# pixray/pixray

Measured on AMD Instinct MI355X. Metric: optimisation iters/sec, VQGAN 256^2 + ViT-B/32 + 64 cutouts, higher is better.
Workload: dtype fp16

## Files before the change

### include/prx.h

```cpp
#ifndef PRX_H_
#define PRX_H_
#include <stddef.h>
#include <stdint.h>

#ifdef __cplusplus
extern "C" {
#endif

#define PRX_ABI_VERSION 3

typedef void* prx_stream_t;

const char* prx_last_error(void);
int prx_abi_version(void);
int prx_device_info(int* cu_count, char* arch_name, int arch_name_len);


#define PRX_ACT_NONE 0
#define PRX_ACT_QUICKGELU 1
#define PRX_ACT_MUL_DQUICKGELU 2
#define PRX_ACT_RELU 3
#define PRX_ACT_MUL_RELUMASK 4
#define PRX_ACT_RELUMASK_POST 5
#define PRX_ACT_GELU 6
// ... 14 lines not shown
    int a_is_f32, a_mode, lda;
    const void* B;
    int ldb;
    int M, N, K;
    int H, W, Cin, up;
    float alpha;
    const float* bias_n;
    const float* bias_m;
    const void* aux;
    int ldaux;
    const float* resid;
    int ldr;
    int act;
    float* out_f32; int ldc_f32;
    void* out_bf16; void* out_bf16_pre; int ldc_bf16;
    int f32;
    int row16;
    prx_gemm_ctx* ctx;
} prx_gemm_args;
int prx_k_gemm(const prx_gemm_args* g, void* ws, size_t ws_bytes, prx_stream_t stream);
int prx_k_gemm_gn(const prx_gemm_args* g, double* gn_stats, int gn_gs, const float* gnb_x, const double* gnb_fstats,
                  const float* gnb_gamma, const float* gnb_beta, int gnb_swish, float gnb_eps, void* ws, size_t ws_bytes,
                  prx_stream_t stream);
long long prx_gemm_fit_spec_launches(void);
long long prx_gemm_row_launches(void);

int prx_k_groupnorm_fwd(const float* x, const float* gamma, const float* beta, double* stats, void* out_bf16,
                        float* out_f32, int NB, int P, int C, int swish, float eps, prx_stream_t s);
int prx_k_groupnorm_bwd(const float* g, const float* x, const float* gamma, const float* beta, const double* fstats,
                        double* bstats, const float* add, float* dx, int NB, int P, int C, int swish, float eps,
                        prx_stream_t s);
int prx_k_layernorm_fwd(const float* x, long long ldx, const float* gamma, const float* beta, void* out_bf16,
                        float* out_f32, float* mean, float* rstd, int rows, int C, float eps, prx_stream_t s);
int prx_k_layernorm_bwd(const float* g, long long ldg, const float* x, long long ldx, const float* gamma,
                        const float* mean, const float* rstd, const float* add, long long ldadd, float* dx,
                        long long lddx, int rows, int C, prx_stream_t s);
int prx_k_transpose_bf16(const void* in, int ldin, void* out, int ldout, int R, int C, prx_stream_t s);
int prx_k_softmax_rows(const float* S, int lds_, float scale, void* P, int ldp, void* PT, int ldpt, int rows, int cols,
                       prx_stream_t s);
int prx_k_softmax_rows_bwd(const void* P, int ldp, const float* dP, int lddp, float scale, void* dS, int ldds,
                           void* dST, int lddst, int rows, int cols, prx_stream_t s);
int prx_k_upsample2x_bwd(const float* hi, float* low, int NB, int Hl, int Wl, int C, prx_stream_t s);
int prx_k_nchw_to_nhwc(const float* in, float* out_f32, void* out_bf16, int NB, int C, int HW, int Cpad,
                       prx_stream_t s);
int prx_k_nhwc_to_nchw(const float* in, int ldc, float* out, int NB, int C, int HW, prx_stream_t s);
int prx_k_image_head_fwd(const float* x, int ldc, float* img, int NB, int C, int HW, prx_stream_t s);
// ... 73 lines not shown
int prx_k_warp_a_bwd(const float* g, int Hs, int Ws, const double* desc, float* uv, float* gsrc_priv, float* gsrc, int n_cut, int Ha,
                     int Wa, int form, prx_stream_t s);
int prx_k_warp_b_fwd(const float* a, int Ha, int Wa, const double* desc, const float* noise, float* out, int n_cut, int S,
                     prx_stream_t s);
int prx_k_warp_b_bwd(const float* a, int Ha, int Wa, const double* desc, const float* g, float* grgb, float* uv, float* ga, int n_cut,
                     int S, float* maps_scratch, size_t maps_scratch_bytes, int form, prx_stream_t s);
int prx_k_vgg_pack(const float* w, void* Wf, void* Wd, int Cout, int Cin, int CiP, int prec, prx_stream_t s);
int prx_k_vgg_input(const float* x, void* out, int HW, int prec, prx_stream_t s);
int prx_k_vgg_input_grad(const float* d, float* gx, int HW, const float* unscale, prx_stream_t s);
int prx_k_vgg_maxpool(const void* x, void* out, void* arg, int H, int W, int C, int prec, prx_stream_t s);
int prx_k_vgg_combine(const float* above, const void* arg, const float* gcap, const void* act, void* gpre, int H, int W, int C,
                      const float* gscale, int prec, prx_stream_t s);
int prx_k_pack_transpose_op(const float* in, void* out, int R, int C, int prec, prx_stream_t s);
int prx_k_vit_add_cls_pos(float* x, const float* cls, const float* pos, int N, int T, int W, prx_stream_t s);
int prx_k_vit_embed_tokens(const float* x, const float* cls, const float* pos, void* out, int out16, int N, int T, int W,
                           prx_stream_t s);
int prx_k_vit_gelu_f32(const float* t, float* io, size_t n, int bwd, prx_stream_t s);
int prx_k_vit_scale_f32(float* x, size_t n, float scale, int blocks, prx_stream_t s);
int prx_k_text_embed(const int* tokens, const float* emb, const float* pos, float* x, int* eot, int n, int ctx, int W, int vocab,
                     prx_stream_t s);
int prx_k_gather_rows(const float* x, const int* eot, float* out, int n, int ctx, int W, prx_stream_t s);
int prx_k_l2norm_fwd(const float* e, float* out, int n, int D, prx_stream_t s);
int prx_k_l2norm_bwd(const float* e, const float* g, float* de, int n, int D, prx_stream_t s);
int prx_k_vqgan_pack_conv3x3(const float* w, void* Wf, void* Wd, int Cout, int Cin, int CoP, int prec, prx_stream_t s);
int prx_k_vqgan_enc_pack_conv3x3(const float* w, void* Wf, int Cout, int Cin, int CiP, prx_stream_t s);
int prx_k_colminmax(const float* w, float* mn, float* mx, int rows, int D, prx_stream_t s);


typedef struct prx_vqgan prx_vqgan;
typedef struct prx_vqgan_config {
    int ch;
    int ch_mult[8];
    int n_mult;
    int num_res_blocks;
    int attn_resolution;
    int resolution;
    int z_channels;
    int embed_dim;
    int n_embed;
    int out_ch;
    int latent_h, latent_w;
    int precision;
} prx_vqgan_config;
int prx_vqgan_create(prx_vqgan** out, const prx_vqgan_config* cfg, const float* const* weights, int n_weights,
                     prx_stream_t s);
void prx_vqgan_destroy(prx_vqgan* h);
// ... 277 lines not shown
```

### pixray_amd/csrc/api_core.hip

```cpp
#include "common.h"
#include "gemm.h"
#include "../../include/prx.h"
#include <stdarg.h>
#include <stdio.h>
#include <string.h>
#include <stdlib.h>

static thread_local char g_err[1024] = "";

void prx_set_error(const char* fmt, ...) {
    va_list ap;
    va_start(ap, fmt);
    vsnprintf(g_err, sizeof(g_err), fmt, ap);
    va_end(ap);
}

int prx_xcd_local() {
    static const int v = getenv("PRX_XCD_LOCAL") ? atoi(getenv("PRX_XCD_LOCAL")) : 1;
    return v;
}

int prx_grad_target_log2() {
    static const int v = [] {
        const char* e = getenv("PRX_GRAD_TARGET_LOG2");
// ... 38 lines not shown
    d.out_f32 = g->out_f32; d.ldc_f32 = g->ldc_f32;
    d.out_bf16 = g->out_bf16; d.out_bf16_pre = g->out_bf16_pre;
    d.ldc_bf16 = g->ldc_bf16;
    d.row16 = (short)(g->row16 & 3);
    return 0;
}
int prx_k_gemm(const prx_gemm_args* g, void* ws, size_t ws_bytes, prx_stream_t stream_) {
    GemmDesc d;
    int r = desc_of(g, d);
    if (r) return r;
    return prx_gemm_launch(d, (float*)ws, ws_bytes, (hipStream_t)stream_, (GemmCtx*)g->ctx);
}
int prx_k_gemm_gn(const prx_gemm_args* g, double* gn_stats, int gn_gs, const float* gnb_x, const double* gnb_fstats,
                  const float* gnb_gamma, const float* gnb_beta, int gnb_swish, float gnb_eps, void* ws, size_t ws_bytes,
                  prx_stream_t stream_) {
    GemmDesc d;
    int r = desc_of(g, d);
    if (r) return r;
    PRX_REQUIRE(gn_stats != nullptr, "prx_k_gemm_gn: null gn_stats");
    d.gn_stats = gn_stats; d.gn_gs = gn_gs;
    d.gnb_x = gnb_x; d.gnb_fstats = gnb_fstats; d.gnb_gamma = gnb_gamma; d.gnb_beta = gnb_beta; d.gnb_swish = gnb_swish; d.gnb_eps = gnb_eps;
    return prx_gemm_launch(d, (float*)ws, ws_bytes, (hipStream_t)stream_, (GemmCtx*)g->ctx);
}

prx_gemm_ctx* prx_gemm_ctx_create(void) { return (prx_gemm_ctx*)new GemmCtx(); }
void prx_gemm_ctx_destroy(prx_gemm_ctx* c) { delete (GemmCtx*)c; }
void prx_profile_gemm_enable(prx_gemm_ctx* c, int on) { prx_gemm_ctx_profile_enable((GemmCtx*)c, on); }
void prx_gemm_tile_override(prx_gemm_ctx* c, int bm, int bn, int splits) { prx_gemm_ctx_force_tile((GemmCtx*)c, bm, bn, splits); }
int prx_gemm_plan(prx_gemm_ctx* c, const prx_gemm_args* g, size_t ws_bytes, int n_cu, int* out) {
    GemmDesc d;
    int r = desc_of(g, d);
    if (r) return r;
    GemmPlan p;
    r = prx_gemm_plan_impl(d, (const GemmCtx*)c, n_cu, ws_bytes, true, &p);
    if (r) return r;
    const GemmLaunchPlan& l0 = p.launch[0], l1 = p.n_launch == 2 ? p.launch[1] : GemmLaunchPlan{};
    const int o[9] = {l0.family, l0.bm, l0.bn, l0.splits, p.rows_8p, p.n_launch == 2 ? (int)l1.family : -1, l1.bm, l1.bn, p.n_launch == 2 ? l1.splits : 0};
    memcpy(out, o, sizeof o);
    return 0;
}
int prx_gemm_plan_rows_8phase(prx_gemm_ctx* c, int M, int N, int K) {
    if (M <= 0 || N <= 0 || K <= 0) return 0;
    prx_gemm_args g = {};
    g.a_mode = PRX_A_ROWMAJOR; g.lda = g.ldb = K; g.M = M; g.N = N; g.K = K; g.alpha = 1.f;
    int out[9];
    return prx_gemm_plan(c, &g, 0, c ? ((GemmCtx*)c)->n_cu : 0, out) == 0 ? out[4] : 0;
// ... 10 lines not shown
```

### pixray_amd/csrc/api_kernels.hip

```cpp
#include "common.h"
#include "norms.h"
#include "elementwise.h"
#include "attention.h"
#include "resnet.h"
#include "cutouts.h"
#include "vgg.h"
#include "vit.h"
#include "clip_text.h"
#include "prompt_vq.h"
#include "vqgan.h"
#include "vqgan_enc.h"
#include "../../include/prx.h"

#define S_(x) ((hipStream_t)(x))
#define B_(x) ((bf16_t*)(x))
#define CB_(x) ((const bf16_t*)(x))

extern "C" {

int prx_k_groupnorm_fwd(const float* x, const float* gamma, const float* beta, double* stats, void* out_bf16,
                        float* out_f32, int NB, int P, int C, int swish, float eps, prx_stream_t s) {
    return prx_groupnorm_fwd(x, gamma, beta, stats, B_(out_bf16), out_f32, NB, P, C, swish, eps, S_(s));
}
int prx_k_groupnorm_bwd(const float* g, const float* x, const float* gamma, const float* beta, const double* fstats,
// ... 272 lines not shown
    return prx_vit_add_cls_pos(x, cls, pos, N, T, W, S_(s));
}
int prx_k_vit_embed_tokens(const float* x, const float* cls, const float* pos, void* out, int out16, int N, int T, int W, prx_stream_t s) {
    return prx_vit_embed_tokens(x, cls, pos, out, out16, N, T, W, S_(s));
}
int prx_k_vit_gelu_f32(const float* t, float* io, size_t n, int bwd, prx_stream_t s) {
    return prx_vit_gelu_f32(t, io, n, bwd, S_(s));
}
int prx_k_vit_scale_f32(float* x, size_t n, float scale, int blocks, prx_stream_t s) {
    return prx_vit_scale_f32(x, n, scale, blocks, S_(s));
}
int prx_k_text_embed(const int* tokens, const float* emb, const float* pos, float* x, int* eot, int n, int ctx, int W, int vocab, prx_stream_t s) {
    return prx_text_embed(tokens, emb, pos, x, eot, n, ctx, W, vocab, S_(s));
}
int prx_k_gather_rows(const float* x, const int* eot, float* out, int n, int ctx, int W, prx_stream_t s) {
    return prx_gather_rows(x, eot, out, n, ctx, W, S_(s));
}
int prx_k_l2norm_fwd(const float* e, float* out, int n, int D, prx_stream_t s) {
    return prx_l2norm_fwd(e, out, n, D, S_(s));
}
int prx_k_l2norm_bwd(const float* e, const float* g, float* de, int n, int D, prx_stream_t s) {
    return prx_l2norm_bwd(e, g, de, n, D, S_(s));
}
int prx_k_vqgan_pack_conv3x3(const float* w, void* Wf, void* Wd, int Cout, int Cin, int CoP, int prec, prx_stream_t s) {
    return prx_vqgan_pack_conv3x3(w, Wf, Wd, Cout, Cin, CoP, prec, S_(s));
}
int prx_k_vqgan_enc_pack_conv3x3(const float* w, void* Wf, int Cout, int Cin, int CiP, prx_stream_t s) {
    return prx_vqgan_enc_pack_conv3x3(w, Wf, Cout, Cin, CiP, S_(s));
}
int prx_k_colminmax(const float* w, float* mn, float* mx, int rows, int D, prx_stream_t s) {
    return prx_colminmax(w, mn, mx, rows, D, S_(s));
}

}
```

### pixray_amd/csrc/gemmfit.hip

```cpp
#include "gemmfit_kernel.h"
#include <atomic>

static std::atomic<long long> g_spec_launches{0};

namespace {
struct FitTile { int bm, bn, ks, tn; double eff; };
const FitTile kFitTiles[] = {
    {160, 256, 1, 64, 1.00}, {160, 192, 1, 48, 0.97}, {256, 128, 1, 64, 0.95}, {160, 128, 1, 32, 0.90}, {128, 128, 1, 32, 0.85},
    {80, 128, 2, 32, 0.85}, {128, 64, 2, 32, 0.75}, {64, 64, 2, 32, 0.60}, {32, 64, 4, 32, 0.45}, {16, 64, 4, 32, 0.35}, {16, 32, 8, 32, 0.25},
    {256, 16, 1, 16, 0.20},
};
const FitTile* fit_tile(int bm, int bn) {
    for (const FitTile& t : kFitTiles)
        if (t.bm == bm && t.bn == bn) return &t;
    return nullptr;
}
}

bool prx_gemmfit_tile(int bm, int bn, int* ks) {
    const FitTile* t = fit_tile(bm, bn);
    if (ks) *ks = t ? t->ks : 0;
    return t != nullptr;
}
bool prx_gemmfit_eligible(const GemmDesc& d, int bm, int bn) {
// ... 48 lines not shown
        if (!prx_gemmfit_eligible(d, tbm, tbn)) return;
        const int tm_ = ceil_div(d.M, tbm), tn_ = ceil_div(d.N, tbn);
        const int wgs = tm_ * tn_;
        if (wgs > 2 * n_cu) return;
        const double fill = (double)wgs / ((double)ceil_div(wgs, n_cu) * n_cu);
        const double waste = ((double)tm_ * tbm / d.M) * ((double)tn_ * tbn / d.N);
        const double score = fill * eff / waste;
        if (score > best && fill / waste >= 0.8) { best = score; *bm = tbm; *bn = tbn; }
    };
    if (d.a_mode == PRX_A_CONV3X3 && d.N <= 16 && d.M >= 4096 && prx_gemmfit_eligible(d, 256, 16)) { *bm = 256; *bn = 16; return; }
    if ((long long)d.M * d.N <= 256ll * 512 && d.K >= 512 && d.N >= 32) {
        if (prx_gemmfit_eligible(d, 16, 32)) { *bm = 16; *bn = 32; return; }
        if (d.N >= 64 && prx_gemmfit_eligible(d, 16, 64)) { *bm = 16; *bn = 64; return; }
    }
    for (const FitTile& t : kFitTiles)
        if (t.bn >= 32) consider(t.bm, t.bn, t.eff);
}
extern std::atomic<long long> g_prx_gemm8p_spec_launches;
extern "C" long long prx_gemm_fit_spec_launches(void) {
    return g_spec_launches.load(std::memory_order_relaxed) + g_prx_gemm8p_spec_launches.load(std::memory_order_relaxed);
}

int prx_gemmfit_epi_kind(const GemmDesc& d) {
    if (!d.h16 || d.f32 || d.a_is_f32 || d.out_f32 || !d.out_bf16 || d.bias_m) return FIT_EPI_GENERIC;
    const unsigned long long lim = 1ull << 31;
    if ((unsigned long long)d.M * d.ldc_bf16 >= lim || (d.resid && (unsigned long long)d.M * d.ldr >= lim) ||
        (d.aux && (unsigned long long)d.M * d.ldaux >= lim) || (unsigned long long)d.M * d.N >= lim) return FIT_EPI_GENERIC;
    const bool stats = d.gn_stats != nullptr, gnb = d.gnb_x != nullptr;
    if (gnb && !stats) return FIT_EPI_GENERIC;
    switch (d.act) {
    case PRX_ACT_NONE:
        if (d.aux) return FIT_EPI_GENERIC;
        if (gnb) return (!d.resid && (d.row16 & 2)) ? FIT_EPI_GNB : FIT_EPI_GENERIC;
        if (d.resid) return (d.row16 & 1) ? (stats ? FIT_EPI_RES16_GN : FIT_EPI_RES16) : FIT_EPI_GENERIC;
        return stats ? FIT_EPI_GN : FIT_EPI_OUT16;
    case PRX_ACT_QUICKGELU:
        return (d.out_bf16_pre && !d.resid && !stats) ? FIT_EPI_GELU : FIT_EPI_GENERIC;
    case PRX_ACT_MUL_DQUICKGELU:
        return (d.aux && !d.resid && !stats) ? FIT_EPI_DGELU : FIT_EPI_GENERIC;
    default:
        return FIT_EPI_GENERIC;
    }
}
#ifdef PRX_FIT_TRACE
namespace {
unsigned long long* g_trace_buf = nullptr;
size_t g_trace_cap = 0, g_trace_used = 0;
// ... 64 lines not shown
```

### pixray_amd/csrc/gemmfit_kernel.h

```cpp
#pragma once
#include "gemm_epi.h"
#include <type_traits>
#include <algorithm>
#include <stdlib.h>
#include <string>
#include <string.h>
#include <stdio.h>

const bf16_t* prx_gemm_zero_page();
int prx_gemmfit_epi_kind(const GemmDesc& d);
bool prx_gemmfit_launch_spec_tower(const prx_gemm_dev::GemmArgs& a, int bm, int bn, int epi, dim3 grid, hipStream_t s, const bf16_t* zp);
bool prx_gemmfit_launch_spec_dec_a(const prx_gemm_dev::GemmArgs& a, int bm, int bn, int epi, dim3 grid, hipStream_t s, const bf16_t* zp);
bool prx_gemmfit_launch_spec_dec_b(const prx_gemm_dev::GemmArgs& a, int bm, int bn, int epi, dim3 grid, hipStream_t s, const bf16_t* zp);
bool prx_gemmfit_launch_spec_dec_c(const prx_gemm_dev::GemmArgs& a, int bm, int bn, int epi, dim3 grid, hipStream_t s, const bf16_t* zp);
bool prx_gemmfit_launch_f32(const prx_gemm_dev::GemmArgs& a, int bm, int bn, dim3 grid, hipStream_t s, const bf16_t* zp);

namespace {
using namespace prx_gemm_dev;

constexpr int FIT_BK = 64;
constexpr int FIT_STAGES = 3;
typedef const __attribute__((address_space(1))) void* fit_gptr;
typedef __attribute__((address_space(3))) void* fit_lptr;

// ... 224 lines not shown
                    fit_gnb_accum(d, gc1, __builtin_bit_cast(float4, pf[ic][ps][1]), v1, gsb0, gsb1);
                } else if (do_stats) {
                    gsa0 += (v0.x + v0.y) + (v0.z + v0.w);
                    gsa1 += (v0.x * v0.x + v0.y * v0.y) + (v0.z * v0.z + v0.w * v0.w);
                    gsb0 += (v1.x + v1.y) + (v1.z + v1.w);
                    gsb1 += (v1.x * v1.x + v1.y * v1.y) + (v1.z * v1.z + v1.w * v1.w);
                }
            }
        }
    }
    FIT_TRACE(5);
    if (do_stats) fit_stats_tail<WGM, WGN, FN, KS>(d, fl + DUMP + 2 * NW * (16 * LDW), gsa0, gsa1, gsb0, gsb1, tn, kg, wm, wn, lane);
}

enum { FIT_EPI_GENERIC = 0,
       FIT_EPI_OUT16,
       FIT_EPI_RES16,
       FIT_EPI_GELU,
       FIT_EPI_DGELU,
       FIT_EPI_GN,
       FIT_EPI_RES16_GN,
       FIT_EPI_GNB,
       FIT_EPI_F32,
       FIT_EPI_COUNT };

__device__ __forceinline__ float fit_sigmoid(float x) { return __builtin_amdgcn_rcpf(1.f + __expf(-x)); }

template <int WGM, int WGN, int FM, int FN, int KS, int EPI>
__device__ __forceinline__ void fit_finish_spec(const GemmArgs& p, float* const fl, f32x4 (&acc)[FM][FN], int tm, int tn, int wave, int kg,
                                                int wt, int wm, int wn, int lane FIT_TRACE_ARG) {
    typedef __attribute__((ext_vector_type(8))) half_t h16x8;
    constexpr int NWT = WGM * WGN, NW = NWT * KS;
    constexpr int BM = 16 * FM * WGM, BN = 16 * FN * WGN, TN = 16 * FN;
    constexpr bool RESID = EPI == FIT_EPI_RES16 || EPI == FIT_EPI_RES16_GN;
    constexpr bool DGELU = EPI == FIT_EPI_DGELU, GELU = EPI == FIT_EPI_GELU, GNB = EPI == FIT_EPI_GNB;
    constexpr bool ROWOP = RESID || DGELU || GNB;
    constexpr bool STATS = EPI == FIT_EPI_GN || EPI == FIT_EPI_RES16_GN || GNB;
    static_assert(!STATS || BM % 80 != 0, "GroupNorm sums belong to the decoder's tiles");
    const GemmDesc& d = p.d;
    const int l15 = lane & 15, kq = lane >> 4;
    constexpr int DUMP = KS > 1 ? NW * FM * FN * 256 : 0;
    fit_ksum<WGM, WGN, FM, FN, KS>(fl, acc, kg, wt, lane);
    FIT_TRACE(4);

    constexpr int LDW = TN + 4, LPR = TN / 8, RPP = 64 / LPR, NPASS = (16 + RPP - 1) / RPP;
    constexpr int NOWN = (FM + KS - 1) / KS;
    constexpr int NBUF = NOWN > 1 ? 2 : 1, SLAB = 16 * LDW;
    float* const stage = fl + DUMP + wave * (2 * SLAB);
    const int rbase = tm * BM + wm * (16 * FM), cbase = tn * BN + wn * TN;
    const int lr0 = lane / LPR, lc = (lane - lr0 * LPR) * 8;
    const int col = cbase + lc;
    const bool col_ok = lane < RPP * LPR && col < d.N;
    const int colc = col_ok ? col : 0;
    const float alpha = d.alpha_dev ? d.alpha * *d.alpha_dev : d.alpha;
    float bias[8] = {0.f, 0.f, 0.f, 0.f, 0.f, 0.f, 0.f, 0.f};
    if (d.bias_n) {
        const float4 b0 = *reinterpret_cast<const float4*>(d.bias_n + colc), b1 = *reinterpret_cast<const float4*>(d.bias_n + colc + 4);
        bias[0] = b0.x; bias[1] = b0.y; bias[2] = b0.z; bias[3] = b0.w; bias[4] = b1.x; bias[5] = b1.y; bias[6] = b1.z; bias[7] = b1.w;
    }
    GnbConst gc0{}, gc1{};
    if constexpr (GNB) { gc0 = gnb_load(d, colc); gc1 = gnb_load(d, colc + 4); }
    const half_t* const rowp = RESID ? reinterpret_cast<const half_t*>(d.resid) : DGELU ? reinterpret_cast<const half_t*>(d.aux)
                                                                                      : reinterpret_cast<const half_t*>(d.gnb_x);
    const unsigned ldrow = RESID ? (unsigned)d.ldr : DGELU ? (unsigned)d.ldaux : (unsigned)d.N;
    half_t* const out = reinterpret_cast<half_t*>(d.out_bf16);
    half_t* const outp = reinterpret_cast<half_t*>(d.out_bf16_pre);
    const unsigned ldo = (unsigned)d.ldc_bf16;
    const int mlast = d.M - 1;

    uint4 pf[ROWOP ? FM : 1][NPASS];
    if constexpr (ROWOP) {
#pragma unroll
        for (int i = 0; i < FM; ++i) {
            if (KS > 1 && i % KS != kg) continue;
#pragma unroll
            for (int ps = 0; ps < NPASS; ++ps) {
                int lr = ps * RPP + lr0;
                lr = lr < 15 ? lr : 15;
                int row = rbase + i * 16 + lr;
                row = row < mlast ? row : mlast;
                pf[i][ps] = *reinterpret_cast<const uint4*>(rowp + ((unsigned)row * ldrow + (unsigned)colc));
            }
        }
    }

    float gsa0 = 0.f, gsa1 = 0.f, gsb0 = 0.f, gsb1 = 0.f;
    auto put = [&](int i, float* st) {
#pragma unroll
        for (int j = 0; j < FN; ++j)
#pragma unroll
// ... 20 lines not shown
                for (int e = 0; e < 8; ++e) x[e] = (float)rx[e];
            }
#pragma unroll
            for (int e = 0; e < 8; ++e) {
                v[e] *= alpha;
                v[e] += bias[e];
                if constexpr (DGELU) {
                    const float sg = fit_sigmoid(1.702f * x[e]);
                    v[e] *= sg * (1.f + 1.702f * x[e] * (1.f - sg));
                }
                if constexpr (RESID) v[e] += x[e];
            }
            const unsigned oo = (unsigned)row * ldo + (unsigned)col;
            if constexpr (GELU) {
                h16x8 q;
#pragma unroll
                for (int e = 0; e < 8; ++e) {
                    q[e] = f32_to_f16_sat(v[e]);
                    const float t = (float)q[e];
                    v[e] = t * fit_sigmoid(1.702f * t);
                }
                if (ok) *reinterpret_cast<h16x8*>(outp + oo) = q;
            }
            {
                h16x8 q;
#pragma unroll
                for (int e = 0; e < 8; ++e) q[e] = f32_to_f16_sat(v[e]);
                if (ok) *reinterpret_cast<h16x8*>(out + oo) = q;
            }
            if constexpr (GNB) {
                if (ok) {
                    fit_gnb_accum<true>(d, gc0, make_float4(x[0], x[1], x[2], x[3]), make_float4(v[0], v[1], v[2], v[3]), gsa0, gsa1);
                    fit_gnb_accum<true>(d, gc1, make_float4(x[4], x[5], x[6], x[7]), make_float4(v[4], v[5], v[6], v[7]), gsb0, gsb1);
                }
            } else if constexpr (STATS) {
                if (ok) {
                    gsa0 += (v[0] + v[1]) + (v[2] + v[3]);
                    gsa1 += (v[0] * v[0] + v[1] * v[1]) + (v[2] * v[2] + v[3] * v[3]);
                    gsb0 += (v[4] + v[5]) + (v[6] + v[7]);
                    gsb1 += (v[4] * v[4] + v[5] * v[5]) + (v[6] * v[6] + v[7] * v[7]);
                }
            }
        }
    }
    FIT_TRACE(5);
    if constexpr (STATS) fit_stats_tail<WGM, WGN, FN, KS>(d, fl + DUMP + 2 * NW * SLAB, gsa0, gsa1, gsb0, gsb1, tn, kg, wm, wn, lane);
}
// ... 424 lines not shown
```

### pixray_amd/csrc/gemmfit_spec_dec_c.hip

```cpp
#include "gemmfit_kernel.h"

#define DEC_TILE(...)                                                                     \
    switch (epi) {                                                                        \
        FIT_SPEC_CASE(FIT_EPI_OUT16, __VA_ARGS__, FIT_EPI_OUT16, true)                    \
        FIT_SPEC_CASE(FIT_EPI_RES16, __VA_ARGS__, FIT_EPI_RES16, true)                    \
        FIT_SPEC_CASE(FIT_EPI_GN, __VA_ARGS__, FIT_EPI_GN, true)                          \
        FIT_SPEC_CASE(FIT_EPI_RES16_GN, __VA_ARGS__, FIT_EPI_RES16_GN, true)              \
        FIT_SPEC_CASE(FIT_EPI_GNB, __VA_ARGS__, FIT_EPI_GNB, true)                        \
        default: return false;                                                            \
    }

bool prx_gemmfit_launch_spec_dec_c(const prx_gemm_dev::GemmArgs& a, int bm, int bn, int epi, dim3 grid, hipStream_t s, const bf16_t* zp) {
    if (bm == 32 && bn == 64) { DEC_TILE(1, 2, 2, 2, 4) }
    if (bm == 16 && bn == 64) { DEC_TILE(1, 2, 1, 2, 4) }
    if (bm == 16 && bn == 32) { DEC_TILE(1, 1, 1, 2, 8) }
    return false;
}
```

### pixray_amd/csrc/gemmfit_spec_tower.hip

```cpp
#include "gemmfit_kernel.h"

#define TOWER_TILE(...)                                                                   \
    switch (epi) {                                                                        \
        FIT_SPEC_CASE(FIT_EPI_OUT16, __VA_ARGS__, FIT_EPI_OUT16, false)                   \
        FIT_SPEC_CASE(FIT_EPI_RES16, __VA_ARGS__, FIT_EPI_RES16, false)                   \
        FIT_SPEC_CASE(FIT_EPI_GELU, __VA_ARGS__, FIT_EPI_GELU, false)                     \
        FIT_SPEC_CASE(FIT_EPI_DGELU, __VA_ARGS__, FIT_EPI_DGELU, false)                   \
        default: return false;                                                            \
    }

bool prx_gemmfit_launch_spec_tower(const prx_gemm_dev::GemmArgs& a, int bm, int bn, int epi, dim3 grid, hipStream_t s, const bf16_t* zp) {
    if (a.d.a_mode != PRX_A_ROWMAJOR) return false;
    if (bm == 160 && bn == 256) { TOWER_TILE(2, 4, 5, 4, 1) }
    if (bm == 160 && bn == 192) { TOWER_TILE(2, 4, 5, 3, 1) }
    if (bm == 160 && bn == 128) { TOWER_TILE(2, 4, 5, 2, 1) }
    if (bm == 80 && bn == 128) { TOWER_TILE(1, 4, 5, 2, 2) }
    return false;
}
```

### pixray_amd/csrc/prompt_vq.h

```cpp
#pragma once
#include "common.h"
int prx_prompt_loss(const float* x, const float* embed, int n, int m, int D, float weight, float stop, float denom,
                    float* rowloss, float* grad, float* loss, unsigned* ticket, hipStream_t s);
int prx_l2norm_fwd(const float* e, float* out, int n, int D, hipStream_t s);
int prx_l2norm_bwd(const float* e, const float* g, float* de, int n, int D, hipStream_t s);
int prx_sqnorm_rows(const float* w, float* out, int rows, int D, hipStream_t s);
int prx_vq_nearest(const float* z, long long tok_stride, long long ch_stride, const float* codebook, const float* cnorm,
                   int P, int NC, int D, float* pmin, int* pidx, int* idx_out, float* zq, hipStream_t s);
```

### pixray_amd/csrc/prompt_vq.hip

```cpp
#include "prompt_vq.h"
#include <algorithm>

namespace {

__device__ __forceinline__ float prompt_loss_row(const float* __restrict__ x, const float* __restrict__ embed, int i, int lane,
                                                int n, int m, int D, float weight, float stop, float denom,
                                                float* __restrict__ rowloss, float* __restrict__ grad) {
    constexpr int MAXE = 16;
    const int ne = D / 64;
    float xv[MAXE], gacc[MAXE];
    float ss = 0.f;
#pragma unroll
    for (int e = 0; e < MAXE; ++e) xv[e] = x[(size_t)i * D + (e < ne ? e : 0) * 64 + lane];
#pragma unroll
    for (int e = 0; e < MAXE; ++e)
        if (e < ne) { ss += xv[e] * xv[e]; gacc[e] = 0.f; }
    const float xnorm = fmaxf(sqrtf(wave_sum(ss)), 1e-12f);
    const float ixn = 1.f / xnorm;
    const float sgn = (weight > 0.f) ? 1.f : ((weight < 0.f) ? -1.f : 0.f);
    float loss = 0.f;
    for (int j = 0; j < m; ++j) {
        float ev[MAXE];
        float es = 0.f;
#pragma unroll
// ... 56 lines not shown
    const int i = blockIdx.x * 4 + (threadIdx.x >> 6);
    if (i >= n) return;
    float ss = 0.f;
    for (int c = lane; c < D; c += 64) { float v = e[(size_t)i * D + c]; ss += v * v; }
    const float inv = 1.f / sqrtf(wave_sum(ss));
    for (int c = lane; c < D; c += 64) out[(size_t)i * D + c] = e[(size_t)i * D + c] * inv;
}
__global__ __launch_bounds__(256) void l2norm_bwd_kernel(const float* __restrict__ e, const float* __restrict__ g,
                                                         float* __restrict__ de, int n, int D) {
    const int lane = threadIdx.x & 63;
    const int i = blockIdx.x * 4 + (threadIdx.x >> 6);
    if (i >= n) return;
    float ss = 0.f, dot = 0.f;
    for (int c = lane; c < D; c += 64) {
        float v = e[(size_t)i * D + c];
        ss += v * v; dot += v * g[(size_t)i * D + c];
    }
    ss = wave_sum(ss); dot = wave_sum(dot);
    const float inv = 1.f / sqrtf(ss);
    for (int c = lane; c < D; c += 64) {
        float v = e[(size_t)i * D + c];
        de[(size_t)i * D + c] = (g[(size_t)i * D + c] - v * dot / ss) * inv;
    }
}

__global__ __launch_bounds__(256) void sqnorm_rows_kernel(const float* __restrict__ w, float* __restrict__ out, int rows, int D) {
    const int lane = threadIdx.x & 63;
    const int i = blockIdx.x * 4 + (threadIdx.x >> 6);
    if (i >= rows) return;
    float ss = 0.f;
    for (int c = lane; c < D; c += 64) { float v = w[(size_t)i * D + c]; ss += v * v; }
    ss = wave_sum(ss);
    if (lane == 0) out[i] = ss;
}

typedef float vq_f32x2 __attribute__((ext_vector_type(2)));
constexpr int VQ_CODES = 128, VQ_CPAD = VQ_CODES + 4;
__global__ __launch_bounds__(256) void vq_dist_kernel(const float* __restrict__ z, long long tok_stride,
                                                      long long ch_stride, const float* __restrict__ codebook,
                                                      const float* __restrict__ cnorm, int P, int NC, int D,
                                                      float* __restrict__ pmin, int* __restrict__ pidx) {
    __shared__ __attribute__((aligned(16))) float Xs[16][64];
    __shared__ __attribute__((aligned(16))) float Cs[16][VQ_CPAD];
    __shared__ float red_v[64][16];
    __shared__ int red_i[64][16];
    const int tid = threadIdx.x;
// ... 108 lines not shown
}

}

int prx_prompt_loss(const float* x, const float* embed, int n, int m, int D, float weight, float stop, float denom,
                    float* rowloss, float* grad, float* loss, unsigned* ticket, hipStream_t s) {
    PRX_REQUIRE(D % 64 == 0 && D <= 1024, "prompt_loss: D must be a multiple of 64 and <= 1024 (D=%d)", D);
    PRX_REQUIRE(!loss || ticket, "prompt_loss: the scalar result needs a zeroed ticket word");
    hipLaunchKernelGGL(prompt_loss_kernel, dim3(ceil_div(n, 4)), dim3(256), 0, s, x, embed, n, m, D, weight, stop, denom,
                       rowloss, grad, loss, ticket);
    PRX_LAUNCH_CHECK();
    return 0;
}
int prx_l2norm_fwd(const float* e, float* out, int n, int D, hipStream_t s) {
    hipLaunchKernelGGL(l2norm_fwd_kernel, dim3(ceil_div(n, 4)), dim3(256), 0, s, e, out, n, D);
    PRX_LAUNCH_CHECK();
    return 0;
}
int prx_l2norm_bwd(const float* e, const float* g, float* de, int n, int D, hipStream_t s) {
    hipLaunchKernelGGL(l2norm_bwd_kernel, dim3(ceil_div(n, 4)), dim3(256), 0, s, e, g, de, n, D);
    PRX_LAUNCH_CHECK();
    return 0;
}
int prx_sqnorm_rows(const float* w, float* out, int rows, int D, hipStream_t s) {
    hipLaunchKernelGGL(sqnorm_rows_kernel, dim3(ceil_div(rows, 4)), dim3(256), 0, s, w, out, rows, D);
    PRX_LAUNCH_CHECK();
    return 0;
}
int prx_vq_nearest(const float* z, long long tok_stride, long long ch_stride, const float* codebook, const float* cnorm,
                   int P, int NC, int D, float* pmin, int* pidx, int* idx_out, float* zq, hipStream_t s) {
    PRX_REQUIRE(D % 16 == 0, "vq: D %% 16 != 0");
    PRX_REQUIRE(((uintptr_t)codebook & 15) == 0, "vq: the codebook must be 16-byte aligned");
    const int ntiles = ceil_div(NC, VQ_CODES);
    hipLaunchKernelGGL(vq_dist_kernel, dim3(ntiles, ceil_div(P, 64)), dim3(256), 0, s, z, tok_stride, ch_stride, codebook,
                       cnorm, P, NC, D, pmin, pidx);
    PRX_LAUNCH_CHECK();
    hipLaunchKernelGGL(vq_select_kernel, dim3(P), dim3(256), 0, s, pmin, pidx, ntiles, codebook, D, idx_out, zq, P);
    PRX_LAUNCH_CHECK();
    return 0;
}
```

### pixray_amd/csrc/vit.hip

```cpp
#include "vit.h"
#include <stdlib.h>
#include "gemm.h"
#include "norms.h"
#include "attention.h"
#include "cutouts.h"
#include "prompt_vq.h"
#include "elementwise.h"
#include "dev_arena.h"
#include <vector>
#include <memory>

namespace {

template <typename TOp>
__global__ __launch_bounds__(256) void pack_transpose_kernel(const float* __restrict__ in, TOp* __restrict__ out,
                                                             int R, int C) {
    __shared__ float tile[32][33];
    const int tx = threadIdx.x & 31, ty = threadIdx.x >> 5;
    const int r0 = blockIdx.y * 32, c0 = blockIdx.x * 32;
#pragma unroll
    for (int i = 0; i < 4; ++i) {
        int r = r0 + ty + 8 * i, c = c0 + tx;
        tile[ty + 8 * i][tx] = (r < R && c < C) ? in[(size_t)r * C + c] : 0.f;
    }
// ... 350 lines not shown
            if ((r = vit_gemm(v, d, s))) return r;
            if (own_pass) {
                if ((r = prx_vit_gelu_f32((const float*)y.t, (float*)v->u, (size_t)rows * 4 * W, 0, s))) return r;
            } }
        {   GemmDesc d; d.A = v->u; d.lda = 4 * W; d.B = y.W2; d.ldb = 4 * W; d.M = rows; d.N = W; d.K = 4 * W;
            d.bias_n = y.b2; d.ldr = ldt;
            if (lean) { d.resid = (const float*)y.x_mid; d.row16 = 1; d.out_bf16 = x_next; d.ldc_bf16 = ldt; }
            else { d.resid = (const float*)y.x_mid; d.out_f32 = (float*)x_next; d.ldc_f32 = ldt; }
            if ((r = vit_gemm(v, d, s))) return r; }
    }
    if ((r = ln_op(v, v->x_final, (long long)T * W, v->lnpost_g, v->lnpost_b, v->hpost, v->mean_post, v->rstd_post, n, s))) return r;
    {   GemmDesc d; d.A = v->hpost; d.lda = W; d.B = v->projT; d.ldb = W; d.M = n; d.N = v->out_dim; d.K = W;
        d.out_f32 = v->e; d.ldc_f32 = v->out_dim;
        if ((r = vit_gemm(v, d, s))) return r; }
    return prx_l2norm_fwd(v->e, embeds, n, v->out_dim, s);
}

int prx_vit_backward_a_impl(PrxVit* v, const float* cutouts, const float* mm, const float* d_embeds, double* acc,
                            hipStream_t s) {
    const int n = v->cur_n;
    PRX_REQUIRE(n >= 1, "vit backward: no forward in flight on this handle");
    const int W = v->width, T = v->T, R = n * T, KP = v->KP, AW = v->aw;
    int r;
    if ((r = prx_l2norm_bwd(v->e, d_embeds, v->de, n, v->out_dim, s))) return r;
    {   GemmDesc d; d.A = v->de; d.a_is_f32 = 1; d.lda = v->out_dim; d.B = v->proj; d.ldb = v->out_dim;
        d.M = n; d.N = W; d.K = v->out_dim; d.out_f32 = v->dhpost; d.ldc_f32 = W;
        if (v->h16) {
            if ((r = prx_grad_scale(v->de, (size_t)n * v->out_dim, v->gs + 2, 64, prx_grad_target_log2(), v->gs, s))) return r;
            if ((r = prx_scale_dev(v->de, (size_t)n * v->out_dim, v->gs, s, (bf16_t*)v->de16, v->h16))) return r;
            d.A = v->de16; d.a_is_f32 = 0;
        }
        if ((r = vit_gemm(v, d, s))) return r; }
    const int lean = v->lean;
    if (v->layers == 0 || !v->cls_tail) PRX_CHECK_HIP(hipMemsetAsync(lean ? v->dx_bf : (void*)v->dx, 0, (lean ? sizeof(bf16_t) : sizeof(float)) * (size_t)R * W, s));
    const void* dxs = lean ? v->dx_bf : (const void*)v->dx;
    const void* dhs = lean ? v->dh_bf : (const void*)v->dh;
    if ((r = ln_bwd_op(v, v->dhpost, W, v->x_final, (long long)T * W, v->lnpost_g, v->mean_post, v->rstd_post,
                       nullptr, 0, v->dx, (long long)T * W, v->dx_bf, n, s, 0, lean ? 1 : 0))) return r;
    for (int l = v->layers - 1; l >= 0; --l) {
        VitLayer& y = v->L[l];
        const bool tail = v->cls_tail && l == v->layers - 1;
        const int rows = tail ? n : R;
        const int ldt = tail ? T * W : W;
        {   GemmDesc d; d.A = v->dx_bf; d.lda = ldt; d.B = y.W2T; d.ldb = W; d.M = rows; d.N = 4 * W; d.K = W;
            d.act = v->fam.dact; d.aux = y.t; d.ldaux = 4 * W; d.out_bf16 = v->dt; d.ldc_bf16 = 4 * W;
            const bool own_pass = v->f32 && v->fam.dact == PRX_ACT_MUL_DGELU;
            if (own_pass) { d.act = PRX_ACT_NONE; d.aux = nullptr; }
            if ((r = vit_gemm(v, d, s))) return r;
            if (own_pass) {
                if ((r = prx_vit_gelu_f32((const float*)y.t, (float*)v->dt, (size_t)rows * 4 * W, 1, s))) return r;
            } }
        {   GemmDesc d; d.A = v->dt; d.lda = 4 * W; d.B = y.W1T; d.ldb = 4 * W; d.M = rows; d.N = W; d.K = 4 * W;
            if (lean) { d.out_bf16 = v->dh_bf; d.ldc_bf16 = W; } else { d.out_f32 = v->dh; d.ldc_f32 = W; }
            if ((r = vit_gemm(v, d, s))) return r; }
// ... 35 lines not shown
```

Before: 163.8.

## Fuse embed-grad l2norm backward, grad scaling and fp16 cast; add fp32-out GEMM epilogue

Replaces three separate launches (l2norm backward, gradient-scale reduction, scale+cast) at the head of the ViT backward with a single one-block kernel for small n*D, and falls back to the old path for larger shapes. Also adds an FIT_EPI_OUT32 epilogue so plain fp16 GEMMs with fp32 output can use the specialised fit kernels instead of the generic path. This removes launch overhead and extra passes over a tiny tensor. The trade-offs are a single-block kernel that serialises the work, and more kernel template instantiations.

```diff
diff --git a/include/prx.h b/include/prx.h
--- a/include/prx.h
+++ b/include/prx.h
@@ -60,6 +60,7 @@
 int prx_k_gemm_gn(const prx_gemm_args* g, double* gn_stats, int gn_gs, const float* gnb_x, const double* gnb_fstats,
                   const float* gnb_gamma, const float* gnb_beta, int gnb_swish, float gnb_eps, void* ws, size_t ws_bytes,
                   prx_stream_t stream);
+int prx_k_gemm_alpha_dev(const prx_gemm_args* g, const float* alpha_dev, void* ws, size_t ws_bytes, prx_stream_t stream);
 long long prx_gemm_fit_spec_launches(void);
 long long prx_gemm_row_launches(void);
 
@@ -179,6 +180,9 @@
 int prx_k_gather_rows(const float* x, const int* eot, float* out, int n, int ctx, int W, prx_stream_t s);
 int prx_k_l2norm_fwd(const float* e, float* out, int n, int D, prx_stream_t s);
 int prx_k_l2norm_bwd(const float* e, const float* g, float* de, int n, int D, prx_stream_t s);
+int prx_k_embed_grad_head(const float* e, const float* g, float* de, void* de16, float* gs, int n, int D, int target_log2, int h16,
+                          prx_stream_t s);
+long long prx_embed_grad_head_launches(void);
 int prx_k_vqgan_pack_conv3x3(const float* w, void* Wf, void* Wd, int Cout, int Cin, int CoP, int prec, prx_stream_t s);
 int prx_k_vqgan_enc_pack_conv3x3(const float* w, void* Wf, int Cout, int Cin, int CiP, prx_stream_t s);
 int prx_k_colminmax(const float* w, float* mn, float* mx, int rows, int D, prx_stream_t s);
diff --git a/pixray_amd/csrc/api_core.hip b/pixray_amd/csrc/api_core.hip
--- a/pixray_amd/csrc/api_core.hip
+++ b/pixray_amd/csrc/api_core.hip
@@ -84,6 +84,13 @@
     d.gnb_x = gnb_x; d.gnb_fstats = gnb_fstats; d.gnb_gamma = gnb_gamma; d.gnb_beta = gnb_beta; d.gnb_swish = gnb_swish; d.gnb_eps = gnb_eps;
     return prx_gemm_launch(d, (float*)ws, ws_bytes, (hipStream_t)stream_, (GemmCtx*)g->ctx);
 }
+int prx_k_gemm_alpha_dev(const prx_gemm_args* g, const float* alpha_dev, void* ws, size_t ws_bytes, prx_stream_t stream_) {
+    GemmDesc d;
+    int r = desc_of(g, d);
+    if (r) return r;
+    d.alpha_dev = alpha_dev;
+    return prx_gemm_launch(d, (float*)ws, ws_bytes, (hipStream_t)stream_, (GemmCtx*)g->ctx);
+}
 
 prx_gemm_ctx* prx_gemm_ctx_create(void) { return (prx_gemm_ctx*)new GemmCtx(); }
 void prx_gemm_ctx_destroy(prx_gemm_ctx* c) { delete (GemmCtx*)c; }
diff --git a/pixray_amd/csrc/api_kernels.hip b/pixray_amd/csrc/api_kernels.hip
--- a/pixray_amd/csrc/api_kernels.hip
+++ b/pixray_amd/csrc/api_kernels.hip
@@ -318,6 +318,10 @@
 int prx_k_l2norm_bwd(const float* e, const float* g, float* de, int n, int D, prx_stream_t s) {
     return prx_l2norm_bwd(e, g, de, n, D, S_(s));
 }
+int prx_k_embed_grad_head(const float* e, const float* g, float* de, void* de16, float* gs, int n, int D, int target_log2, int h16,
+                          prx_stream_t s) {
+    return prx_embed_grad_head(e, g, de, B_(de16), gs, n, D, target_log2, h16, S_(s));
+}
 int prx_k_vqgan_pack_conv3x3(const float* w, void* Wf, void* Wd, int Cout, int Cin, int CoP, int prec, prx_stream_t s) {
     return prx_vqgan_pack_conv3x3(w, Wf, Wd, Cout, Cin, CoP, prec, S_(s));
 }
diff --git a/pixray_amd/csrc/gemmfit.hip b/pixray_amd/csrc/gemmfit.hip
--- a/pixray_amd/csrc/gemmfit.hip
+++ b/pixray_amd/csrc/gemmfit.hip
@@ -94,7 +94,11 @@
 }
 
 int prx_gemmfit_epi_kind(const GemmDesc& d) {
-    if (!d.h16 || d.f32 || d.a_is_f32 || d.out_f32 || !d.out_bf16 || d.bias_m) return FIT_EPI_GENERIC;
+    if (!d.h16 || d.f32 || d.a_is_f32 || d.bias_m) return FIT_EPI_GENERIC;
+    if (d.out_f32 && !d.out_bf16 && !d.out_bf16_pre && d.act == PRX_ACT_NONE && !d.resid && !d.aux && !d.gn_stats && !d.gnb_x &&
+        (unsigned long long)d.M * d.ldc_f32 < (1ull << 31))
+        return FIT_EPI_OUT32;
+    if (d.out_f32 || !d.out_bf16) return FIT_EPI_GENERIC;
     const unsigned long long lim = 1ull << 31;
     if ((unsigned long long)d.M * d.ldc_bf16 >= lim || (d.resid && (unsigned long long)d.M * d.ldr >= lim) ||
         (d.aux && (unsigned long long)d.M * d.ldaux >= lim) || (unsigned long long)d.M * d.N >= lim) return FIT_EPI_GENERIC;
diff --git a/pixray_amd/csrc/gemmfit_kernel.h b/pixray_amd/csrc/gemmfit_kernel.h
--- a/pixray_amd/csrc/gemmfit_kernel.h
+++ b/pixray_amd/csrc/gemmfit_kernel.h
@@ -270,6 +270,7 @@
        FIT_EPI_RES16_GN,
        FIT_EPI_GNB,
        FIT_EPI_F32,
+       FIT_EPI_OUT32,
        FIT_EPI_COUNT };
 
 __device__ __forceinline__ float fit_sigmoid(float x) { return __builtin_amdgcn_rcpf(1.f + __expf(-x)); }
@@ -282,6 +283,7 @@
     constexpr int BM = 16 * FM * WGM, BN = 16 * FN * WGN, TN = 16 * FN;
     constexpr bool RESID = EPI == FIT_EPI_RES16 || EPI == FIT_EPI_RES16_GN;
     constexpr bool DGELU = EPI == FIT_EPI_DGELU, GELU = EPI == FIT_EPI_GELU, GNB = EPI == FIT_EPI_GNB;
+    constexpr bool OUT32 = EPI == FIT_EPI_OUT32;
     constexpr bool ROWOP = RESID || DGELU || GNB;
     constexpr bool STATS = EPI == FIT_EPI_GN || EPI == FIT_EPI_RES16_GN || GNB;
     static_assert(!STATS || BM % 80 != 0, "GroupNorm sums belong to the decoder's tiles");
@@ -313,7 +315,8 @@
     const unsigned ldrow = RESID ? (unsigned)d.ldr : DGELU ? (unsigned)d.ldaux : (unsigned)d.N;
     half_t* const out = reinterpret_cast<half_t*>(d.out_bf16);
     half_t* const outp = reinterpret_cast<half_t*>(d.out_bf16_pre);
-    const unsigned ldo = (unsigned)d.ldc_bf16;
+    const unsigned ldo = OUT32 ? (unsigned)d.ldc_f32 : (unsigned)d.ldc_bf16;
+    float* const out32 = d.out_f32;
     const int mlast = d.M - 1;
 
     uint4 pf[ROWOP ? FM : 1][NPASS];
@@ -380,7 +383,12 @@
                 }
                 if (ok) *reinterpret_cast<h16x8*>(outp + oo) = q;
             }
-            {
+            if constexpr (OUT32) {
+                if (ok) {
+                    *reinterpret_cast<float4*>(out32 + oo) = make_float4(v[0], v[1], v[2], v[3]);
+                    *reinterpret_cast<float4*>(out32 + oo + 4) = make_float4(v[4], v[5], v[6], v[7]);
+                }
+            } else {
                 h16x8 q;
 #pragma unroll
                 for (int e = 0; e < 8; ++e) q[e] = f32_to_f16_sat(v[e]);
diff --git a/pixray_amd/csrc/gemmfit_spec_dec_c.hip b/pixray_amd/csrc/gemmfit_spec_dec_c.hip
--- a/pixray_amd/csrc/gemmfit_spec_dec_c.hip
+++ b/pixray_amd/csrc/gemmfit_spec_dec_c.hip
@@ -10,7 +10,17 @@
         default: return false;                                                            \
     }
 
+#define DEC_TILE_OUT32(...)                                                               \
+    if (epi == FIT_EPI_OUT32) {                                                           \
+        if (a.d.a_mode != PRX_A_ROWMAJOR) return false;                                   \
+        launch_fit_spec<__VA_ARGS__, FIT_EPI_OUT32, false>(a, grid, s, zp);               \
+        return true;                                                                      \
+    }
+
 bool prx_gemmfit_launch_spec_dec_c(const prx_gemm_dev::GemmArgs& a, int bm, int bn, int epi, dim3 grid, hipStream_t s, const bf16_t* zp) {
+    if (bm == 32 && bn == 64) { DEC_TILE_OUT32(1, 2, 2, 2, 4) }
+    if (bm == 16 && bn == 64) { DEC_TILE_OUT32(1, 2, 1, 2, 4) }
+    if (bm == 16 && bn == 32) { DEC_TILE_OUT32(1, 1, 1, 2, 8) }
     if (bm == 32 && bn == 64) { DEC_TILE(1, 2, 2, 2, 4) }
     if (bm == 16 && bn == 64) { DEC_TILE(1, 2, 1, 2, 4) }
     if (bm == 16 && bn == 32) { DEC_TILE(1, 1, 1, 2, 8) }
diff --git a/pixray_amd/csrc/gemmfit_spec_tower.hip b/pixray_amd/csrc/gemmfit_spec_tower.hip
--- a/pixray_amd/csrc/gemmfit_spec_tower.hip
+++ b/pixray_amd/csrc/gemmfit_spec_tower.hip
@@ -9,8 +9,13 @@
         default: return false;                                                            \
     }
 
+#define TOWER_TILE_OUT32(...)                                                             \
+    if (epi == FIT_EPI_OUT32) { launch_fit_spec<__VA_ARGS__, FIT_EPI_OUT32, false>(a, grid, s, zp); return true; }
+
 bool prx_gemmfit_launch_spec_tower(const prx_gemm_dev::GemmArgs& a, int bm, int bn, int epi, dim3 grid, hipStream_t s, const bf16_t* zp) {
     if (a.d.a_mode != PRX_A_ROWMAJOR) return false;
+    if (bm == 160 && bn == 256) { TOWER_TILE_OUT32(2, 4, 5, 4, 1) }
+    if (bm == 80 && bn == 128) { TOWER_TILE_OUT32(1, 4, 5, 2, 2) }
     if (bm == 160 && bn == 256) { TOWER_TILE(2, 4, 5, 4, 1) }
     if (bm == 160 && bn == 192) { TOWER_TILE(2, 4, 5, 3, 1) }
     if (bm == 160 && bn == 128) { TOWER_TILE(2, 4, 5, 2, 1) }
diff --git a/pixray_amd/csrc/prompt_vq.h b/pixray_amd/csrc/prompt_vq.h
--- a/pixray_amd/csrc/prompt_vq.h
+++ b/pixray_amd/csrc/prompt_vq.h
@@ -4,6 +4,9 @@
                     float* rowloss, float* grad, float* loss, unsigned* ticket, hipStream_t s);
 int prx_l2norm_fwd(const float* e, float* out, int n, int D, hipStream_t s);
 int prx_l2norm_bwd(const float* e, const float* g, float* de, int n, int D, hipStream_t s);
+constexpr long long PRX_EMBED_GRAD_HEAD_MAX = 65536;
+int prx_embed_grad_head(const float* e, const float* g, float* de, bf16_t* de16, float* gs, int n, int D, int target_log2, int h16,
+                        hipStream_t s);
 int prx_sqnorm_rows(const float* w, float* out, int rows, int D, hipStream_t s);
 int prx_vq_nearest(const float* z, long long tok_stride, long long ch_stride, const float* codebook, const float* cnorm,
                    int P, int NC, int D, float* pmin, int* pidx, int* idx_out, float* zq, hipStream_t s);
diff --git a/pixray_amd/csrc/prompt_vq.hip b/pixray_amd/csrc/prompt_vq.hip
--- a/pixray_amd/csrc/prompt_vq.hip
+++ b/pixray_amd/csrc/prompt_vq.hip
@@ -1,5 +1,7 @@
 #include "prompt_vq.h"
+#include "elementwise.h"
 #include <algorithm>
+#include <atomic>
 
 namespace {
 
@@ -102,6 +104,53 @@
         float v = e[(size_t)i * D + c];
         de[(size_t)i * D + c] = (g[(size_t)i * D + c] - v * dot / ss) * inv;
     }
+}
+
+__global__ __launch_bounds__(1024) void embed_grad_head_kernel(const float* __restrict__ e, const float* __restrict__ g, float* __restrict__ de,
+                                                               bf16_t* __restrict__ de16, float* __restrict__ gs, int n, int D,
+                                                               int target_log2, int chain_blocks, int h16) {
+    const int lane = threadIdx.x & 63, wave = threadIdx.x >> 6;
+    float m = 0.f, m0 = 0.f;
+    for (int i = wave; i < n; i += 16) {
+        float ss = 0.f, dot = 0.f;
+        for (int c = lane; c < D; c += 64) {
+            float v = e[(size_t)i * D + c];
+            ss += v * v; dot += v * g[(size_t)i * D + c];
+        }
+        ss = wave_sum(ss); dot = wave_sum(dot);
+        const float inv = 1.f / sqrtf(ss);
+        for (int c = lane; c < D; c += 64) {
+            float v = e[(size_t)i * D + c];
+            const float x = (g[(size_t)i * D + c] - v * dot / ss) * inv;
+            de[(size_t)i * D + c] = x;
+            float a = fabsf(x);
+            a = a == a ? a : INFINITY;
+            m = fmaxf(m, a);
+            if ((((unsigned)(i * D + c)) >> 8) % (unsigned)chain_blocks == 0) m0 = fmaxf(m0, a);
+        }
+    }
+    m = wave_max(m); m0 = wave_max(m0);
+    __shared__ float sm[16], sm0[16];
+    if (lane == 0) { sm[wave] = m; sm0[wave] = m0; }
+    __syncthreads();
+    m = sm[0]; m0 = sm0[0];
+#pragma unroll
+    for (int w = 1; w < 16; ++w) { m = fmaxf(m, sm[w]); m0 = fmaxf(m0, sm0[w]); }
+    float S = 1.f;
+    if (m > 0.f && m < INFINITY) {
+        int ex;
+        (void)frexpf(m, &ex);
+        int k = target_log2 - ex;
+        k = k < -40 ? -40 : (k > 60 ? 60 : k);
+        S = ldexpf(1.f, k);
+    }
+    if (threadIdx.x == 0) { gs[0] = S; gs[1] = 1.f / S; gs[2] = m0; }
+    for (int i = wave; i < n; i += 16)
+        for (int c = lane; c < D; c += 64) {
+            const float v = de[(size_t)i * D + c] * S;
+            de[(size_t)i * D + c] = v;
+            de16[(size_t)i * D + c] = to_op16(v, h16);
+        }
 }
 
 __global__ __launch_bounds__(256) void sqnorm_rows_kernel(const float* __restrict__ w, float* __restrict__ out, int rows, int D) {
@@ -256,6 +305,23 @@
     PRX_LAUNCH_CHECK();
     return 0;
 }
+static std::atomic<long long> g_head_launches{0};
+extern "C" long long prx_embed_grad_head_launches(void) { return g_head_launches.load(std::memory_order_relaxed); }
+int prx_embed_grad_head(const float* e, const float* g, float* de, bf16_t* de16, float* gs, int n, int D, int target_log2, int h16,
+                        hipStream_t s) {
+    PRX_REQUIRE(n >= 1 && D >= 1 && (long long)n * D < (1ll << 31), "embed_grad_head: bad shape %d x %d", n, D);
+    if ((long long)n * D > PRX_EMBED_GRAD_HEAD_MAX) {
+        int r;
+        if ((r = prx_l2norm_bwd(e, g, de, n, D, s))) return r;
+        if ((r = prx_grad_scale(de, (size_t)n * D, gs + 2, 64, target_log2, gs, s))) return r;
+        return prx_scale_dev(de, (size_t)n * D, gs, s, de16, h16);
+    }
+    g_head_launches.fetch_add(1, std::memory_order_relaxed);
+    const int chain_blocks = (int)std::min<size_t>(((size_t)n * D + 1023) / 1024 + 1, (size_t)64);
+    hipLaunchKernelGGL(embed_grad_head_kernel, dim3(1), dim3(1024), 0, s, e, g, de, de16, gs, n, D, target_log2, chain_blocks, h16);
+    PRX_LAUNCH_CHECK();
+    return 0;
+}
 int prx_sqnorm_rows(const float* w, float* out, int rows, int D, hipStream_t s) {
     hipLaunchKernelGGL(sqnorm_rows_kernel, dim3(ceil_div(rows, 4)), dim3(256), 0, s, w, out, rows, D);
     PRX_LAUNCH_CHECK();
diff --git a/pixray_amd/csrc/vit.hip b/pixray_amd/csrc/vit.hip
--- a/pixray_amd/csrc/vit.hip
+++ b/pixray_amd/csrc/vit.hip
@@ -396,14 +396,11 @@
     PRX_REQUIRE(n >= 1, "vit backward: no forward in flight on this handle");
     const int W = v->width, T = v->T, R = n * T, KP = v->KP, AW = v->aw;
     int r;
-    if ((r = prx_l2norm_bwd(v->e, d_embeds, v->de, n, v->out_dim, s))) return r;
+    if (v->h16) { if ((r = prx_embed_grad_head(v->e, d_embeds, v->de, (bf16_t*)v->de16, v->gs, n, v->out_dim, prx_grad_target_log2(), v->h16, s))) return r; }
+    else if ((r = prx_l2norm_bwd(v->e, d_embeds, v->de, n, v->out_dim, s))) return r;
     {   GemmDesc d; d.A = v->de; d.a_is_f32 = 1; d.lda = v->out_dim; d.B = v->proj; d.ldb = v->out_dim;
         d.M = n; d.N = W; d.K = v->out_dim; d.out_f32 = v->dhpost; d.ldc_f32 = W;
-        if (v->h16) {
-            if ((r = prx_grad_scale(v->de, (size_t)n * v->out_dim, v->gs + 2, 64, prx_grad_target_log2(), v->gs, s))) return r;
-            if ((r = prx_scale_dev(v->de, (size_t)n * v->out_dim, v->gs, s, (bf16_t*)v->de16, v->h16))) return r;
-            d.A = v->de16; d.a_is_f32 = 0;
-        }
+        if (v->h16) { d.A = v->de16; d.a_is_f32 = 0; }
         if ((r = vit_gemm(v, d, s))) return r; }
     const int lean = v->lean;
     if (v->layers == 0 || !v->cls_tail) PRX_CHECK_HIP(hipMemsetAsync(lean ? v->dx_bf : (void*)v->dx, 0, (lean ? sizeof(bf16_t) : sizeof(float)) * (size_t)R * W, s));
```

New measurement: 164.5 (median of 6 runs). No clear change (+0.4%).
